# goroda/GPEXP

Hardware: AMD Instinct MI355X
Metric: GP-fit+IVAR-eval points/s at N=32768 d=8 (wall-time in ms_per_step); value = (N+M)/t_step, SURVEY 8d's N/t_fit and M/t_IVAR are points_per_s_fit / points_per_s_ivar right behind it (higher is better)
Workload: dtype f64; 1 GPU; C4: N=32768 d=8 Matern-5/2 (rho=0.5,s=1,noise=0.1) kfill+potrf+potrs+logdet+IVAR over M=32768 MC points; N=32768, d=8, M=32768, kernel=matern52, seed=32768, parallelism=1 GPU

## Files before the change

### gpexp_amd/_lib.py

```python
import ctypes as C
import os

import numpy as np

_HERE = os.path.dirname(os.path.abspath(__file__))
LIB_PATH = os.path.join(_HERE, "libgpx_hip.so")

c_i64 = C.c_int64
c_dp = C.POINTER(C.c_double)
c_ip = C.POINTER(c_i64)
c_vp = C.c_void_p

_SIGS = {
    "gpx_abi_version": (C.c_int, []),
    "gpx_last_error": (C.c_char_p, []),
    "gpx_create": (C.c_int, [C.c_int, C.POINTER(c_vp)]),
    "gpx_destroy": (C.c_int, [c_vp]),
    "gpx_sync": (C.c_int, [c_vp]),
    "gpx_trim": (C.c_int, [c_vp]),
    "gpx_device_info": (C.c_int, [c_vp, C.c_char_p, C.c_int, C.POINTER(C.c_int), c_ip, C.POINTER(C.c_int)]),
    "gpx_mat_from_host": (C.c_int, [c_vp, c_dp, c_i64, c_i64, C.c_int, C.POINTER(c_vp)]),
    "gpx_mat_alloc": (C.c_int, [c_vp, c_i64, c_i64, C.c_int, C.POINTER(c_vp)]),
    "gpx_mat_free": (C.c_int, [c_vp, c_vp]),
    "gpx_mat_clone": (C.c_int, [c_vp, c_vp, C.POINTER(c_vp)]),
# ... 113 lines not shown
    "gpx_dist2_diag_pack": (C.c_int, [c_vp, c_vp, c_i64, c_i64, c_i64, c_vp, c_i64, c_i64]),
    "gpx_dist2_update": (C.c_int, [c_vp, c_vp, c_i64, c_i64, c_i64, c_i64, c_vp, c_i64, c_i64, c_i64, c_i64]),
    "gpx_dist2_update_multi": (C.c_int, [c_vp, c_vp, c_i64, c_i64, c_i64, c_i64, c_i64, C.c_int, C.c_int, C.c_int, C.c_int, c_i64,
                                         C.c_int, C.POINTER(c_vp), c_ip, C.c_int]),
    "gpx_dist2_pack_rows": (C.c_int, [c_vp, c_vp, c_i64, c_i64, c_i64, c_vp, c_i64, c_i64, c_i64, c_i64]),
    "gpx_dist2_pack_diag": (C.c_int, [c_vp, c_vp, c_i64, c_i64, c_i64, c_vp, c_i64]),
    "gpx_program_run": (C.c_int, [c_vp, c_ip, c_i64, c_ip, c_i64, c_dp]),
    "gpx_program_capture": (C.c_int, [c_vp, c_ip, c_i64, c_ip, c_i64, C.POINTER(c_vp)]),
    "gpx_graph_launch": (C.c_int, [c_vp, c_vp, c_dp, c_ip]),
    "gpx_graph_free": (C.c_int, [c_vp, c_vp]),
    "gpx_dist2_unpack_rows": (C.c_int, [c_vp, c_vp, c_i64, c_i64, c_i64, c_i64, c_vp, c_i64, c_i64, c_i64]),
    "gpx_dist2_unpack_diag": (C.c_int, [c_vp, c_vp, c_i64, c_i64, c_i64, c_vp, c_i64]),
    "gpx_dist2_unpack_diag_at": (C.c_int, [c_vp, c_vp, c_i64, c_i64, c_i64, c_vp, c_i64, c_i64]),
    "gpx_dist2_trsv_diag": (C.c_int, [c_vp, c_vp, c_i64, c_i64, c_i64, c_vp, c_i64, C.c_int]),
    "gpx_dist2_gemv": (C.c_int, [c_vp, c_vp, c_i64, c_i64, c_i64, c_i64, c_vp, c_i64, c_vp, c_i64, C.c_int]),
    "gpx_dist2_logdet_acc": (C.c_int, [c_vp, c_vp, c_i64, c_i64, c_i64, c_i64, c_vp]),
    "gpx_stream_select": (C.c_int, [c_vp, C.c_int]),
    "gpx_event_record": (C.c_int, [c_vp, C.c_int]),
    "gpx_event_wait": (C.c_int, [c_vp, C.c_int]),
    "gpx_dist_finish": (C.c_int, [c_vp, c_vp]),
    "gpx_ivar_grad": (C.c_int, [c_vp, C.c_int, C.c_int, c_dp, C.c_int, c_vp, c_vp, c_vp, c_dp, c_dp]),
    "gpx_ivar_grad_w": (C.c_int, [c_vp, C.c_int, C.c_int, c_dp, C.c_int, c_vp, c_vp, c_vp, c_dp, c_vp, c_dp]),
    "gpx_ivar_grad_rows": (C.c_int, [c_vp, C.c_int, C.c_int, c_dp, C.c_int, c_vp, c_vp, c_vp, c_vp, c_i64, c_dp]),
    "gpx_var_grad": (C.c_int, [c_vp, C.c_int, C.c_int, c_dp, C.c_int, c_vp, c_vp, c_vp, c_dp, c_dp, c_dp, c_dp]),
    "gpx_var_grad_newpt": (C.c_int, [c_vp, C.c_int, C.c_int, c_dp, C.c_int, c_vp, c_vp, c_vp, c_dp]),
    "gpx_fitc_var_grad": (C.c_int, [c_vp, c_vp, C.c_int, C.c_int, c_dp, C.c_int, c_vp, c_vp, c_dp, c_dp, c_dp, c_dp]),
    "gpx_fitc_var_grad_newpt": (C.c_int, [c_vp, c_vp, C.c_int, C.c_int, c_dp, C.c_int, c_vp, c_vp, c_dp]),
    "gpx_profile_enable": (C.c_int, [c_vp, C.c_int]),
    "gpx_profile_reset": (C.c_int, [c_vp]),
    "gpx_profile_get": (C.c_int, [c_vp, C.c_int, c_ip, c_dp, c_dp, c_dp]),
    "gpx_dbg_gemm": (C.c_int, [c_vp, c_vp, c_vp, c_vp, C.c_int, C.c_int, C.c_int]),
    "gpx_dbg_gemm_strassen": (C.c_int, [c_vp, c_vp, c_vp, c_vp]),
    "gpx_dbg_gemm_strassen_depth": (C.c_int, [c_vp, c_vp, c_vp, c_vp, C.c_int]),
    "gpx_dbg_gemm_tri": (C.c_int, [c_vp, c_vp, c_vp, c_vp, C.c_int, C.c_int, C.c_int]),
    "gpx_dbg_gemm_ksplit": (C.c_int, [c_vp, c_vp, c_vp, c_vp, C.c_int, C.c_int]),
    "gpx_dbg_kfill_plan": (C.c_int, [c_vp, C.c_int, C.c_int, c_dp, C.c_int, c_vp, c_vp, C.POINTER(C.c_int), c_dp]),
    "gpx_dbg_colreduce_plan": (C.c_int, [c_i64, c_i64, C.POINTER(c_i64), C.POINTER(c_i64)]),
    "gpx_dbg_panel_bcast_plan": (C.c_int, [C.c_int, C.c_int, c_i64, C.c_int, C.POINTER(c_i64), C.POINTER(C.c_int),
                                           C.POINTER(c_i64), c_i64, C.POINTER(c_i64)]),
    "gpx_dbg_guard_violations": (c_i64, [c_vp]),
    "gpx_dbg_guard_selftest": (C.c_int, [c_vp]),
    "gpx_dbg_pool_stats": (C.c_int, [c_vp, C.POINTER(c_i64), C.POINTER(c_i64)]),
    "gpx_dbg_spin": (C.c_int, [c_vp, C.c_int]),
    "gpx_dbg_spin_us": (C.c_int, [c_vp, c_i64]),
    "gpx_dbg_stamp": (C.c_int, [c_vp, C.c_int]),
    "gpx_dbg_spin_until": (C.c_int, [c_vp, C.c_int, c_i64]),
    "gpx_dbg_event_elapsed": (C.c_int, [c_vp, C.c_int, C.c_int, c_dp]),
    "gpx_dbg_leaf_stamps": (C.c_int, [c_vp, c_vp, C.c_int, C.POINTER(c_i64)]),
    "gpx_dbg_greedy_var_scores": (C.c_int, [c_vp, C.c_int, C.c_int, c_dp, C.c_int, c_vp, c_ip, c_i64, c_dp]),
}

_lib = None


def load():
    global _lib
    if _lib is not None:
        return _lib
    path = os.environ.get("GPX_LIB_PATH", LIB_PATH)
    if not os.path.exists(path):
        raise ImportError(
            "gpexp_amd: %s not found - the HIP library is required (no CPU fallback). "
            "Build it with `make -C gpexp_amd/csrc` or __graft_entry__.build()." % path)
    lib = C.CDLL(path)
    for name, (res, args) in _SIGS.items():
        fn = getattr(lib, name)
# ... 43 lines not shown
```

### gpexp_amd/csrc/api.hip

```cpp
#include "gpx_internal.h"
#include <stdarg.h>
#include <stdio.h>
#include <string.h>
#include <math.h>
#include <stdlib.h>

static thread_local char g_err[1024] = "";

void gpx_set_error(const char* fmt, ...) {
  va_list ap;
  va_start(ap, fmt);
  vsnprintf(g_err, sizeof(g_err), fmt, ap);
  va_end(ap);
}

static constexpr int64_t GUARD = 4096;

int gpx_dev_alloc(gpx_ctx* ctx, int64_t bytes, void** out) {
  if (bytes <= 0) bytes = 8;
  bytes = gpx_round_up(bytes, 256);
  const int64_t key = bytes + (ctx->guard ? 2 * GUARD : 0);
  void* base = nullptr;
  auto it = ctx->pool.find(key);
  if (it != ctx->pool.end()) {
// ... 1327 lines not shown
                   : launch_gemm_ksplit_small(ctx, A->p, A->ld, B->p, B->ld, C->p, C->ld, m, n, k, mode == 3, parts, P);
}

int gpx_dbg_gemm(gpx_ctx* ctx, const gpx_mat* A, const gpx_mat* B, gpx_mat* C, int bt, int accumulate, int lower) {
  GPX_ARG(ctx && A && B && C, "NULL argument");
  const int64_t m = C->prows, n = C->pcols, k = A->pcols;
  GPX_ARG(A->prows == m, "A rows");
  GPX_ARG(bt ? (B->prows == n && B->pcols == k) : (B->prows == k && B->pcols == n), "B shape");
  GPX_TRY(launch_gemm(ctx, A->p, A->ld, B->p, B->ld, C->p, C->ld, m, n, k, bt != 0, accumulate != 0,
                      lower != 0));
  GPX_HIP(hipStreamSynchronize(ctx->stream));
  return 0;
}

int gpx_dbg_gemm_strassen(gpx_ctx* ctx, const gpx_mat* A, const gpx_mat* B, gpx_mat* C) {
  GPX_ARG(ctx && A && B && C, "NULL argument");
  const int64_t m = C->prows, n = C->pcols, k = A->pcols;
  GPX_ARG(A->prows == m && B->prows == k && B->pcols == n, "operand shapes");
  GPX_TRY(launch_gemm_strassen(ctx, A->p, A->ld, B->p, B->ld, C->p, C->ld, m, n, k, 1, nullptr, 0));
  GPX_HIP(hipStreamSynchronize(ctx->stream));
  return 0;
}

int gpx_dbg_gemm_strassen_depth(gpx_ctx* ctx, const gpx_mat* A, const gpx_mat* B, gpx_mat* C, int depth) {
  GPX_ARG(ctx && A && B && C, "NULL argument");
  GPX_ARG(depth >= 0 && depth <= GPX_STRASSEN_MAX_DEPTH, "strassen: depth out of range");
  const int64_t m = C->prows, n = C->pcols, k = A->pcols;
  GPX_ARG(A->prows == m && B->prows == k && B->pcols == n, "operand shapes");
  GPX_TRY(launch_gemm_strassen(ctx, A->p, A->ld, B->p, B->ld, C->p, C->ld, m, n, k, depth, nullptr, 0));
  GPX_HIP(hipStreamSynchronize(ctx->stream));
  return 0;
}

}
```

### gpexp_amd/csrc/chol.hip

```cpp
#include "gpx_internal.h"
#include <algorithm>
#include <math.h>
#include <stdlib.h>
#include <stddef.h>

namespace {

constexpr int NB = GPX_TILE;
constexpr int LS = NB + 1;

typedef double d4 __attribute__((ext_vector_type(4)));

__device__ __forceinline__ double readlane_d(double v, int srclane) {
  int lo = __builtin_amdgcn_readlane(__double2loint(v), srclane);
  int hi = __builtin_amdgcn_readlane(__double2hiint(v), srclane);
  return __hiloint2double(hi, lo);
}

constexpr int LB = 16;
constexpr int TS17 = LB + 1;
constexpr int BSZ = LB * TS17;
constexpr int LEAF_CB = LB * LB + 64 + LB;

__device__ __forceinline__ constexpr int sb_off(int I, int J) { return (I * (I + 1) / 2 + J) * BSZ; }
// ... 1249 lines not shown
  const int64_t mid = (b0 + b1) / 2;
  GPX_TRY(trsm_left_oop_rec(ctx, P, b0, mid, B, ldb, W, ldw, m));
  const int64_t r0 = blk_off(P, mid), r1 = blk_off(P, b1), c0 = blk_off(P, b0);
  const int depth = P.strassen ? std::min(P.strassen, strassen_gate(r1 - r0, m, r0 - c0)) : 0;
  if (depth > 0)
    GPX_TRY(launch_gemm_strassen(ctx, P.L + r0 * P.ld + c0, P.ld, W + c0 * ldw, ldw, B + r0 * ldb, ldb, r1 - r0, m, r0 - c0,
                                 depth, P.sscr, P.sscr_bytes));
  else
    GPX_TRY(launch_gemm(ctx, P.L + r0 * P.ld + c0, P.ld, W + c0 * ldw, ldw, B + r0 * ldb, ldb, r1 - r0, m, r0 - c0, false,
                        true, false));
  return trsm_left_oop_rec(ctx, P, mid, b1, B, ldb, W, ldw, m);
}

int chol_trsm_left_oop(gpx_ctx* ctx, gpx_mat* Lm, double* B, int64_t ldb, double* W, int64_t ldw, int64_t m) {
  GPX_ARG(Lm && Lm->factored && Lm->aux && B && W && B != W, "trsm: matrix has not been factored / bad buffers");
  if (m == 0) return 0;
  GPX_TRY(chol_binv_ensure(ctx, Lm));
  PotrsPlan P;
  P.L = Lm->p;
  P.ld = Lm->ld;
  P.n = Lm->prows;
  P.sib = Lm->binv_ib;
  P.ib = P.sib < 1024 ? P.sib : 1024;
  P.nblk = (P.n + P.ib - 1) / P.ib;
  P.binv = Lm->binv;
  P.binvT = nullptr;
  P.part = nullptr;
  void* ps = nullptr;
  int64_t sbytes = 0;
  int depth = 0;
  const int64_t max_depth = env_i64("GPX_STRASSEN", GPX_STRASSEN_MAX_DEPTH);
  if (P.nblk >= 2 && max_depth > 0) {
    const int64_t r0 = blk_off(P, P.nblk / 2);
    for (depth = (int)std::min<int64_t>(max_depth, strassen_gate(P.n - r0, m, r0)); depth > 0; --depth) {
      sbytes = gemm_strassen_scratch_bytes(P.n - r0, m, r0, depth);
      if (sbytes > 0 && gpx_dev_alloc(ctx, sbytes, &ps) == 0) break;
      (void)hipGetLastError();
      ps = nullptr;
    }
  }
  P.strassen = ps ? depth : 0;
  P.sscr = (double*)ps;
  P.sscr_bytes = sbytes;
  const int r = trsm_left_oop_rec(ctx, P, 0, P.nblk, B, ldb, W, ldw, m);
  if (ps) {
    (void)hipStreamSynchronize(ctx->stream);
    gpx_dev_release(ctx, ps, sbytes);
  }
  return r;
}

int chol_trsm_left_group(gpx_ctx* ctx, const double* Lg, int64_t ld, const double* invd, int64_t w, int64_t below, int64_t ib,
                         double* B, int64_t ldb, int64_t m, double* inv, double* tmp, double* W, int64_t ldw) {
  GPX_ARG(Lg && invd && B && inv && tmp && W && W != B && w > 0 && w % NB == 0 && ib >= NB && ib % NB == 0, "trsm group: bad arguments");
  if (m == 0) return 0;
  GPX_TRY(binv_build_range(ctx, Lg, ld, invd, inv, ib, w, tmp));
  PotrsPlan P;
  P.L = Lg;
  P.ld = ld;
  P.n = w;
  P.ib = P.sib = ib;
  P.nblk = (w + ib - 1) / ib;
  P.binv = inv;
  P.binvT = nullptr;
  P.part = nullptr;
  GPX_TRY(trsm_left_oop_rec(ctx, P, 0, P.nblk, B, ldb, W, ldw, m));
  if (below > 0) GPX_TRY(launch_gemm(ctx, Lg + w * ld, ld, W, ldw, B + w * ldb, ldb, below, m, w, false, true, false));
  return gpx_copy2d(ctx, W, ldw, B, ldb, w, m);
}
// ... 66 lines not shown
```

### gpexp_amd/csrc/gemm_f64.hip

```cpp
#include "gpx_internal.h"
#include <stdlib.h>

namespace {

typedef double d4 __attribute__((ext_vector_type(4)));

constexpr int KB = 16;
constexpr int SA = KB + 1;

template <bool BT, int TE>
struct Smem {
  double a[2][TE * SA];
  double b[2][BT ? TE * SA : KB * (TE + 16)];
};

template <bool LOWER>
__device__ __forceinline__ bool tile_of(int sblk, int within, int tiles_m, int tiles_n, int sb_cols, int sb_shift,
                                        int* by, int* bx, int rot = 0) {
  const int sbm = (1 << sb_shift) - 1;
  int sr, sc;
  if (LOWER) {
    const int nsr = (tiles_m + sbm) >> sb_shift;
    const int noff = nsr * (nsr - 1) / 2;
    if (sblk < noff) {
// ... 397 lines not shown
  gemm_tile<false, true, TE, NoSeg, Multi>(sm, A, lda, B, ldb, dst.c[0], ldc, nk, by, bx, NoSeg(), dst);
}

template <bool BSIDE>
__global__ __launch_bounds__(256) void strassen_sums_kernel(const double* __restrict__ X, int64_t ldx, int64_t hr, int64_t hc,
                                                            double* __restrict__ S, int64_t lds, int64_t sstride) {
  const int64_t j = ((int64_t)blockIdx.x * 256 + threadIdx.x) * 2;
  if (j >= hc) return;
  for (int64_t i = blockIdx.y; i < hr; i += gridDim.y) {
    const double* x1 = X + i * ldx + j;
    const double* x2 = X + (i + hr) * ldx + j;
    const double2 x11 = *reinterpret_cast<const double2*>(x1);
    const double2 x12 = *reinterpret_cast<const double2*>(x1 + hc);
    const double2 x21 = *reinterpret_cast<const double2*>(x2);
    const double2 x22 = *reinterpret_cast<const double2*>(x2 + hc);
    double* o = S + i * lds + j;
#define GPX_S2(k_, ex_, ey_) *reinterpret_cast<double2*>(o + (k_) * sstride) = make_double2(ex_, ey_)
    GPX_S2(0, x11.x + x22.x, x11.y + x22.y);
    if (BSIDE) {
      GPX_S2(1, x12.x - x22.x, x12.y - x22.y);
      GPX_S2(2, x21.x - x11.x, x21.y - x11.y);
      GPX_S2(3, x11.x + x12.x, x11.y + x12.y);
      GPX_S2(4, x21.x + x22.x, x21.y + x22.y);
    } else {
      GPX_S2(1, x21.x + x22.x, x21.y + x22.y);
      GPX_S2(2, x11.x + x12.x, x11.y + x12.y);
      GPX_S2(3, x21.x - x11.x, x21.y - x11.y);
      GPX_S2(4, x12.x - x22.x, x12.y - x22.y);
    }
#undef GPX_S2
  }
}

template <bool BT, bool ACC>
__global__ __launch_bounds__(256, 2) void gemm_f64_batched_kernel(const double* A, int64_t lda, int64_t sa,
                                                                  const double* B, int64_t ldb, int64_t sb, double* C,
                                                                  int64_t ldc, int64_t sc, int nk, int tiles_n, int hiprio) {
  __shared__ Smem<BT, 64> sm;
  if (hiprio) __builtin_amdgcn_s_setprio(3);
  const int64_t b = blockIdx.y;
  const int by = blockIdx.x / tiles_n, bx = blockIdx.x - by * tiles_n;
  gemm_tile<BT, ACC, 64>(sm, A + b * sa, lda, B + b * sb, ldb, C + b * sc, ldc, nk, by, bx);
}

template <bool LOWER>
__global__ __launch_bounds__(256, 2) void gemm_f64_ksplit_kernel(const double* A, int64_t lda, const double* B, int64_t ldb,
                                                                 double* P, int64_t n, int64_t sp, int nk_slice, int parts,
                                                                 int tiles_m, int tiles_n, int sb_cols, int sb_shift) {
  __shared__ Smem<true, 128> sm;
  const int w = blockIdx.x, xcd = w & 7, q = w >> 3, sbs2 = 2 * sb_shift;
  const int job = (q >> sbs2) * 8 + xcd, within = q & ((1 << sbs2) - 1);
  int sb, slice;
  if (LOWER) {
    const int nsr = (tiles_m + (1 << sb_shift) - 1) >> sb_shift, noff = nsr * (nsr - 1) / 2;
    if (job < parts * noff) {
      slice = job / noff;
      sb = job - slice * noff;
    } else {
      const int jj = job - parts * noff;
      slice = jj / nsr;
      sb = noff + jj - slice * nsr;
    }
  } else {
    const int nsb = ((tiles_m + (1 << sb_shift) - 1) >> sb_shift) * sb_cols;
    slice = job / nsb;
    sb = job - slice * nsb;
// ... 273 lines not shown
  return 0;
}

static int launch_gemm_multi(gpx_ctx* ctx, const double* A, int64_t lda, const double* B, int64_t ldb, const Multi& dst,
                             int64_t ldc, int64_t m, int64_t n, int64_t k) {
  GPX_ARG(m % 128 == 0 && n % 128 == 0 && k % KB == 0 && k > 0 && m > 0 && n > 0, "gemm: m,n must be multiples of 128 and k of 16");
  GPX_ARG((lda % 2) == 0 && (ldb % 2) == 0, "gemm: leading dimensions must be even (16-byte loads)");
  GPX_ARG(dst.nd >= 1 && dst.nd <= GPX_MULTI_MAX, "gemm: bad destination count");
  const double tiles128 = (double)(m / 128) * (double)(n / 128);
  const int te = tiles128 < 1024.0 ? 64 : 128;
  const Plan p = make_plan(m, n, false, te);
  GPX_ARG(p.wgs < ((int64_t)1 << 31), "gemm: grid too large");
  const int nk = (int)(k / KB);
  ProfScope ps(ctx, GPX_PROF_GEMM, 2.0 * (double)m * (double)n * (double)k, 0.0);
  if (te == 64)
    hipLaunchKernelGGL(gemm_f64_multi_kernel<64>, dim3((unsigned)p.wgs), dim3(256), 0, ctx->stream, A, lda, B, ldb, dst, ldc, nk,
                       p.tm, p.tn, p.sbc, p.sb_shift);
  else
    hipLaunchKernelGGL(gemm_f64_multi_kernel<128>, dim3((unsigned)p.wgs), dim3(256), 0, ctx->stream, A, lda, B, ldb, dst, ldc, nk,
                       p.tm, p.tn, p.sbc, p.sb_shift);
  GPX_HIP(hipGetLastError());
  return 0;
}

static inline bool strassen_shape_ok(int64_t m, int64_t n, int64_t k, int depth) {
  return depth >= 1 && depth <= GPX_STRASSEN_MAX_DEPTH && m > 0 && n > 0 && k > 0 && m % ((int64_t)128 << depth) == 0 &&
         n % ((int64_t)128 << depth) == 0 && k % ((int64_t)KB << depth) == 0;
}

static inline int64_t strassen_level_elems(int64_t hm, int64_t hn, int64_t hk) {
  return 5 * (hm * gpx_skew_ld(hk) + hk * gpx_skew_ld(hn));
}

int64_t gemm_strassen_scratch_bytes(int64_t m, int64_t n, int64_t k, int depth) {
  if (!strassen_shape_ok(m, n, k, depth)) return 0;
  int64_t elems = 0;
  for (int d = 0; d < depth; ++d) {
    m /= 2, n /= 2, k /= 2;
    elems += strassen_level_elems(m, n, k);
  }
  return elems * 8;
}

namespace {
struct SDest {
  double* c;
  double s;
};
struct SProd {
  int a, b, nq, q[2];
  double s[2];
};
constexpr SProd kStrassen[7] = {
    {-1, -1, 2, {0, 3}, {1.0, 1.0}},
    {-2, 0, 2, {2, 3}, {1.0, -1.0}},
    {0, -2, 2, {1, 3}, {1.0, 1.0}},
    {3, -3, 2, {0, 2}, {1.0, 1.0}},
    {-3, 3, 2, {1, 0}, {1.0, -1.0}},
    {-4, -4, 1, {3, 0}, {1.0, 0.0}},
    {-5, -5, 1, {0, 0}, {1.0, 0.0}},
};
}

static int strassen_rec(gpx_ctx* ctx, const double* A, int64_t lda, const double* B, int64_t ldb, const SDest* dst, int nd,
                        int64_t ldc, int64_t m, int64_t n, int64_t k, int depth, double* scratch) {
  if (depth == 0) {
    for (int d = 1; d < nd; ++d)
      for (int e = 0; e < d; ++e) GPX_ARG(dst[d].c != dst[e].c, "strassen: two destinations of one product coincide");
    if (nd == 1 && dst[0].s == 1.0) return launch_gemm(ctx, A, lda, B, ldb, dst[0].c, ldc, m, n, k, false, true, false);
    if (nd == 2 && dst[0].s == 1.0) return launch_gemm_dual(ctx, A, lda, B, ldb, dst[0].c, dst[1].c, dst[1].s, ldc, m, n, k);
    GPX_ARG(nd >= 1 && nd <= GPX_MULTI_MAX, "strassen: too many destinations for one product");
    Multi md;
    for (int d = 0; d < GPX_MULTI_MAX; ++d) {
      md.c[d] = d < nd ? dst[d].c : nullptr;
      md.s[d] = d < nd ? dst[d].s : 0.0;
    }
    md.nd = nd;
    return launch_gemm_multi(ctx, A, lda, B, ldb, md, ldc, m, n, k);
  }
  const int64_t hm = m / 2, hn = n / 2, hk = k / 2, lsa = gpx_skew_ld(hk), lsb = gpx_skew_ld(hn);
  const int64_t sa = hm * lsa, sb = hk * lsb;
  double* const S = scratch;
  double* const T = scratch + 5 * sa;
  double* const below = T + 5 * sb;
  {
    ProfScope ps(ctx, GPX_PROF_REDUCE, 5.0 * (double)hm * hk + 5.0 * (double)hk * hn, 72.0 * ((double)hm * hk + (double)hk * hn));
    hipLaunchKernelGGL(strassen_sums_kernel<false>, dim3((unsigned)((hk / 2 + 255) / 256), (unsigned)(hm < 65535 ? hm : 65535)),
                       dim3(256), 0, ctx->stream, A, lda, hm, hk, S, lsa, sa);
    hipLaunchKernelGGL(strassen_sums_kernel<true>, dim3((unsigned)((hn / 2 + 255) / 256), (unsigned)(hk < 65535 ? hk : 65535)),
                       dim3(256), 0, ctx->stream, B, ldb, hk, hn, T, lsb, sb);
    if (hipGetLastError() != hipSuccess) {
      gpx_set_error("strassen: operand-sum launch failed");
      return -2;
    }
  }
  const int64_t qoff[4] = {0, hn, hm * ldc, hm * ldc + hn};
  for (const SProd& p : kStrassen) {
    const double* Ap = p.a < 0 ? S + (-1 - p.a) * sa : (p.a == 0 ? A : A + hm * lda + hk);
    const double* Bp = p.b < 0 ? T + (-1 - p.b) * sb : (p.b == 0 ? B : B + hk * ldb + hn);
    SDest sub[GPX_MULTI_MAX];
    int ns = 0;
    for (int d = 0; d < nd; ++d)
      for (int j = 0; j < p.nq; ++j) {
        GPX_ARG(ns < GPX_MULTI_MAX, "strassen: too many destinations for one product");
        sub[ns++] = SDest{dst[d].c + qoff[p.q[j]], dst[d].s * p.s[j]};
      }
    GPX_TRY(strassen_rec(ctx, Ap, p.a < 0 ? lsa : lda, Bp, p.b < 0 ? lsb : ldb, sub, ns, ldc, hm, hn, hk, depth - 1, below));
  }
  return 0;
}

int launch_gemm_strassen(gpx_ctx* ctx, const double* A, int64_t lda, const double* B, int64_t ldb, double* C, int64_t ldc,
                         int64_t m, int64_t n, int64_t k, int depth, double* scratch, int64_t scratch_bytes) {
  if (depth > GPX_STRASSEN_MAX_DEPTH) depth = GPX_STRASSEN_MAX_DEPTH;
  if ((lda % 2) != 0 || (ldb % 2) != 0 || C == A || C == B) depth = 0;
  void* own = nullptr;
  int64_t need = 0;
  for (; depth > 0; --depth) {
    need = gemm_strassen_scratch_bytes(m, n, k, depth);
    if (need == 0) continue;
    if (scratch && scratch_bytes >= need) break;
    if (gpx_dev_alloc(ctx, need, &own) == 0) {
      scratch = (double*)own;
      break;
    }
    (void)hipGetLastError();
    own = nullptr;
  }
  if (depth <= 0) return launch_gemm(ctx, A, lda, B, ldb, C, ldc, m, n, k, false, true, false);
  const SDest top{C, 1.0};
  const int r = strassen_rec(ctx, A, lda, B, ldb, &top, 1, ldc, m, n, k, depth, scratch);
  if (own) {
    (void)hipStreamSynchronize(ctx->stream);
    gpx_dev_release(ctx, own, need);
  }
  return r;
}

int launch_dist2_update(gpx_ctx* ctx, double* C, int64_t ldc, int64_t lr0, int64_t m, int64_t lc0, int64_t n, int64_t nb, int Pr,
                        int Pc, int pr, int pc, int64_t piece_stride, int64_t dsz, int nseg, const double* const* g,
                        const int64_t* ks, int below_diag) {
  if (m == 0 || n == 0 || nseg == 0) return 0;
  GPX_ARG(nseg > 0 && nseg <= GPX_SEG_MAX && Pr >= 1 && Pr <= GPX_MAX_PR && Pc >= 1, "dist2 update: too many segments / grid rows");
  GPX_ARG(m % 128 == 0 && n % 128 == 0 && nb % 128 == 0 && lr0 % nb == 0 && lc0 % nb == 0 && (ldc % 2) == 0, "dist2 update: alignment");
  Dist2Upd u;
  for (int s = 0; s < nseg; ++s) {
    u.g[s] = g[s];
    for (int p = 0; p < Pr; ++p) u.li0[s][p] = (int)(ks[s] + 1 <= p ? 0 : (ks[s] - p) / Pr + 1);
  }
  u.nseg = nseg;
  u.seg_nk = (int)(nb / KB);
  u.Pr = Pr; u.Pc = Pc; u.pr = pr; u.pc = pc;
  u.nb = (int)nb;
  u.gld = (int)gpx_g_ld(nb);
  u.li_first = (int)(lr0 / nb);
  u.lj_first = (int)(lc0 / nb);
  u.below_diag = below_diag;
  u.piece_stride = piece_stride;
  u.dsz = dsz;
  double tiles128 = 0.0;
  for (int64_t lj = lc0 / nb; lj * nb < lc0 + n; ++lj) {
    const int64_t J = lj * Pc + pc;
    const int64_t cw = (lc0 + n - lj * nb) < nb ? (lc0 + n - lj * nb) : nb;
    for (int64_t li = lr0 / nb; li * nb < lr0 + m; ++li) {
// ... 56 lines not shown
```

### gpexp_amd/csrc/gpx_internal.h

```cpp
#pragma once
#include <hip/hip_runtime.h>
#include <stdint.h>
#include <stdlib.h>
#include <string>
#include <vector>
#include <map>
#include <memory>
#include <unordered_set>
#include "../../include/gpx.h"
#include "../../include/gpx_dist.h"
#include "../../include/gpx_debug.h"

#define GPX_TILE 128
#define GPX_MAXD GPX_MAX_DIM
#define GPX_NSTREAMS 6
#define GPX_SEG_MAX 8
#ifndef GPX_G_SKEW
#define GPX_G_SKEW 0
#endif
#define GPX_MAX_PR 4

void gpx_set_error(const char* fmt, ...);
#define GPX_HIP(call)                                                                   \
  do {                                                                                  \
// ... 215 lines not shown
    else if ((kind_) == GPX_K_MATERN32) GPX_SE_DISPATCH(GPX_K_MATERN32, d_, CALL); \
    else GPX_SE_DISPATCH(GPX_K_MATERN52, d_, CALL);                             \
  } while (0)

extern "C" __attribute__((visibility("hidden"))) int64_t gpx_eval_chunk(int64_t np);
int gpx_posterior_chunk(gpx_ctx* ctx, const KParams& kp, const gpx_mat* L, const gpx_mat* X, const double* Zc, int64_t mc,
                        double* B, double* Wout, const double* alpha_dev, double* mean_dev, double* mean_host, double* ssq,
                        double* kd, double* part);

int launch_kfill(gpx_ctx* ctx, const KParams& kp, const double* A, int64_t na, const double* B, int64_t nb,
                 int symmetric, const double* d_nugget, int64_t nugget_len, double nugget_scalar,
                 double* out, int64_t prows, int64_t pcols, int64_t ld);
int launch_kfill_offset(gpx_ctx* ctx, const KParams& kp, const double* X, int64_t n, int64_t row_off, int64_t col_off,
                        const double* d_nugget, int64_t nugget_len, double nugget_scalar, double* out, int64_t prows,
                        int64_t pcols, int64_t ld);
int launch_kdiag(gpx_ctx* ctx, const KParams& kp, const double* Z, int64_t m, double* out);
int launch_kfill_cyclic(gpx_ctx* ctx, const KParams& kp, const double* X, int64_t n, const double* d_nugget,
                        int64_t nugget_len, double nugget_scalar, double* out, int64_t prows, int64_t pcols, int64_t ld,
                        int64_t nb, int Pr, int pr, int Pc, int pc);
int gpx_copy2d(gpx_ctx* ctx, const double* src, int64_t lds_, double* dst, int64_t ldd, int64_t rows, int64_t cols);
int gpx_copy2d_lower(gpx_ctx* ctx, const double* src, int64_t lds_, double* dst, int64_t ldd, int64_t n);
int launch_kfill_rows(gpx_ctx* ctx, const KParams& kp, const double* X, int64_t n, int64_t row0, const double* d_nugget,
                      int64_t nugget_len, double nugget_scalar, double* out, int64_t prows_band, int64_t pcols,
                      int64_t ld);

static inline int gpx_chain_prio(const gpx_ctx* ctx) { return ctx->stream == ctx->streams[1] ? 1 : 0; }
int launch_gemm(gpx_ctx* ctx, const double* A, int64_t lda, const double* B, int64_t ldb, double* C, int64_t ldc,
                int64_t m, int64_t n, int64_t k, bool bt, bool accumulate, bool lower);

int launch_gemm_tri(gpx_ctx* ctx, const double* A, int64_t lda, const double* B, int64_t ldb, double* C, int64_t ldc,
                    int64_t m, int64_t n, int64_t k, bool bt, bool accumulate, bool lower, int tri);
constexpr int GPX_STRASSEN_MAX_DEPTH = 2;
int64_t gemm_strassen_scratch_bytes(int64_t m, int64_t n, int64_t k, int depth);
int launch_gemm_strassen(gpx_ctx* ctx, const double* A, int64_t lda, const double* B, int64_t ldb, double* C, int64_t ldc,
                         int64_t m, int64_t n, int64_t k, int depth, double* scratch, int64_t scratch_bytes);
int launch_gemm_ksplit(gpx_ctx* ctx, const double* A, int64_t lda, const double* B, int64_t ldb, double* C, int64_t ldc,
                       int64_t m, int64_t n, int64_t k, bool lower, int64_t parts, double* P, bool assign = false);
int launch_gemm_ksplit_small(gpx_ctx* ctx, const double* A, int64_t lda, const double* B, int64_t ldb, double* C, int64_t ldc,
                             int64_t m, int64_t n, int64_t k, bool assign, int64_t parts, double* P);
int launch_gemm_batched(gpx_ctx* ctx, const double* A, int64_t lda, int64_t sa, const double* B, int64_t ldb, int64_t sb,
                        double* C, int64_t ldc, int64_t sc, int64_t m, int64_t n, int64_t k, bool bt, bool accumulate,
                        int64_t batch);

int launch_dist2_update(gpx_ctx* ctx, double* C, int64_t ldc, int64_t lr0, int64_t m, int64_t lc0, int64_t n, int64_t nb, int Pr,
                        int Pc, int pr, int pc, int64_t piece_stride, int64_t dsz, int nseg, const double* const* g,
                        const int64_t* ks, int below_diag);

int launch_leaf(gpx_ctx* ctx, double* A, int64_t ld, double* inv, int64_t base_index, int64_t n_valid);
int chol_potrf(gpx_ctx* ctx, double* A, int64_t ld, int64_t n, double* invd, int64_t n_valid);
int chol_potrf_nozero(gpx_ctx* ctx, double* A, int64_t ld, int64_t n, double* invd, int64_t base, int64_t n_valid);
int chol_trsm_right(gpx_ctx* ctx, const double* L, int64_t ldl, const double* invd, double* X, int64_t ldx,
                    int64_t m, int64_t n);
int chol_trsm_right_n(gpx_ctx* ctx, const double* L, int64_t ldl, const double* invd, double* X, int64_t ldx,
                      int64_t m, int64_t n);
int chol_trsm_left(gpx_ctx* ctx, const double* L, int64_t ldl, const double* invd, double* B, int64_t ldb,
                   int64_t n, int64_t m);
int chol_trsv(gpx_ctx* ctx, const double* L, int64_t ld, const double* invd, double* y, int64_t n, bool transposed);
int64_t chol_trsv_scratch_bytes(int64_t n);
int chol_trsv_with_scratch(gpx_ctx* ctx, const double* L, int64_t ld, const double* invd, double* y, int64_t n,
                           bool transposed, double* scratch);
int launch_logdet(gpx_ctx* ctx, const double* L, int64_t ld, int64_t n, double* d_out);
int chol_trtri(gpx_ctx* ctx, const gpx_mat* L, double* Linv, double* tmp);
int chol_binv_ensure(gpx_ctx* ctx, gpx_mat* L);
int chol_trsm_right_trailing(gpx_ctx* ctx, gpx_mat* L, int64_t r0, double* X, int64_t ldx, int64_t m, int transposed, double* T);
int chol_trsm_right_leading(gpx_ctx* ctx, gpx_mat* L, int64_t ncols, double* X, int64_t ldx, int64_t m, double* T, int64_t tcap);
int chol_trsm_right_n_leading(gpx_ctx* ctx, gpx_mat* L, int64_t ncols, double* X, int64_t ldx, int64_t m, double* T);
// ... 49 lines not shown
```

### gpexp_amd/device.py

```python
import ctypes as C
import atexit
import os

import numpy as np

from . import _lib
from ._lib import check, as_f64, dptr, c_vp, c_i64, GpxError

K_SE, K_MATERN32, K_MATERN52, K_MEHLER = 0, 1, 2, 3
PROF_CLASSES = ["kfill", "gemm", "leaf", "trsv", "reduce", "greedy", "comm", "kcross"]

_ctx = None


class Context:

    def __init__(self, device=None):
        self.lib = _lib.load()
        if device is None:
            device = int(os.environ.get("LOCAL_RANK", "0"))
        h = c_vp()
        rc = self.lib.gpx_create(int(device), C.byref(h))
        if rc != 0:
            raise RuntimeError("gpexp_amd needs an MI355X: " + self.lib.gpx_last_error().decode())
# ... 769 lines not shown


def var_grad_newpt(ctx, spec, L, X, Z):
    out = np.empty(Z.shape[0] * spec.d)
    check(ctx.lib.gpx_var_grad_newpt(ctx.h, *spec.args(), L.h, X.h, Z.h, dptr(out)))
    return out


def kfill_plan(ctx, spec, X, Z=None):
    ex = C.c_int()
    cen = np.zeros(spec.d)
    check(ctx.lib.gpx_dbg_kfill_plan(ctx.h, *spec.args(), X.h, Z.h if Z is not None else None, C.byref(ex), dptr(cen)))
    return bool(ex.value), cen


def dbg_gemm_tri(ctx, A, B, Cm, bt, accumulate, tri):
    check(ctx.lib.gpx_dbg_gemm_tri(ctx.h, A.h, B.h, Cm.h, int(bt), int(accumulate), int(tri)))


def dbg_gemm_ksplit(ctx, A, B, Cm, mode, parts):
    check(ctx.lib.gpx_dbg_gemm_ksplit(ctx.h, A.h, B.h, Cm.h, int(mode), int(parts)))


def dbg_gemm(ctx, A, B, Cm, bt, accumulate, lower=False):
    check(ctx.lib.gpx_dbg_gemm(ctx.h, A.h, B.h, Cm.h, int(bt), int(accumulate), int(lower)))


def dbg_gemm_strassen(ctx, A, B, Cm):
    check(ctx.lib.gpx_dbg_gemm_strassen(ctx.h, A.h, B.h, Cm.h))


def dbg_gemm_strassen_depth(ctx, A, B, Cm, depth):
    check(ctx.lib.gpx_dbg_gemm_strassen_depth(ctx.h, A.h, B.h, Cm.h, int(depth)))
```

### include/gpx_debug.h

```cpp
#ifndef GPX_DEBUG_H
#define GPX_DEBUG_H
#include "gpx.h"
#ifdef __cplusplus
extern "C" {
#endif

int gpx_dbg_gemm(gpx_ctx* ctx, const gpx_mat* A, const gpx_mat* B, gpx_mat* C, int bt, int accumulate, int lower);
int gpx_dbg_gemm_tri(gpx_ctx* ctx, const gpx_mat* A, const gpx_mat* B, gpx_mat* C, int bt, int accumulate, int tri);
int gpx_dbg_gemm_ksplit(gpx_ctx* ctx, const gpx_mat* A, const gpx_mat* B, gpx_mat* C, int mode, int parts);
int gpx_dbg_gemm_strassen(gpx_ctx* ctx, const gpx_mat* A, const gpx_mat* B, gpx_mat* C);
int gpx_dbg_gemm_strassen_depth(gpx_ctx* ctx, const gpx_mat* A, const gpx_mat* B, gpx_mat* C, int depth);
int gpx_dbg_spin(gpx_ctx* ctx, int ms);
int64_t gpx_dbg_guard_violations(gpx_ctx* ctx);
int gpx_dbg_pool_stats(gpx_ctx* ctx, int64_t* pooled_bytes, int64_t* outstanding_bytes);
int gpx_dbg_guard_selftest(gpx_ctx* ctx);
int gpx_dbg_panel_bcast_plan(int W, int me, int64_t small_elems, int npieces, const int64_t* counts, const int* roots,
                             int64_t* ops, int64_t max_ops, int64_t* nops);
int gpx_dbg_colreduce_plan(int64_t rows, int64_t pcols, int64_t* nchunk, int64_t* bound_elems);
int gpx_dbg_kfill_plan(gpx_ctx* ctx, int kind, int d, const double* hyp, int nhyp, const gpx_mat* X, const gpx_mat* Z,
                       int* exact, double* center);

int gpx_dbg_spin_us(gpx_ctx* ctx, int64_t us);
int gpx_dbg_stamp(gpx_ctx* ctx, int slot);
int gpx_dbg_spin_until(gpx_ctx* ctx, int slot, int64_t us);
int gpx_dbg_event_elapsed(gpx_ctx* ctx, int id0, int id1, double* ms);

int gpx_dbg_leaf_stamps(gpx_ctx* ctx, gpx_mat* K, int fast, int64_t* out30);

int gpx_dbg_greedy_var_scores(gpx_ctx* ctx, int kind, int d, const double* hyp, int nhyp, const gpx_mat* C, const int64_t* keep,
                              int64_t nkeep, double* out_d );

#ifdef __cplusplus
}
#endif
#endif
```

Measured before the change: 105,300 points/s.

## Add one-pass depth-2 Strassen that precomputes all operand sums in one kernel

Adds a one-pass form of two-level Strassen. A single kernel per operand computes all 45 quarter-block sums of A and B up front, then the 49 leaf products run directly from those sums, replacing the recursive two-pass scheme with its intermediate level. A ladder picks the first form whose scratch fits, and it is used in the potrs trsm and the strassen gemm path. The one-pass form needs more scratch memory (45 quarter blocks per operand), so it falls back to two-pass or plain gemm when allocation fails.

```diff
diff --git a/gpexp_amd/_lib.py b/gpexp_amd/_lib.py
--- a/gpexp_amd/_lib.py
+++ b/gpexp_amd/_lib.py
@@ -169,6 +169,11 @@
     "gpx_dbg_gemm": (C.c_int, [c_vp, c_vp, c_vp, c_vp, C.c_int, C.c_int, C.c_int]),
     "gpx_dbg_gemm_strassen": (C.c_int, [c_vp, c_vp, c_vp, c_vp]),
     "gpx_dbg_gemm_strassen_depth": (C.c_int, [c_vp, c_vp, c_vp, c_vp, C.c_int]),
+    "gpx_dbg_gemm_strassen_view": (C.c_int, [c_vp, c_vp, c_i64, c_i64, c_vp, c_i64, c_i64, c_vp, c_i64, c_i64, c_i64, c_i64, c_i64,
+                                             C.c_int]),
+    "gpx_dbg_strassen_forms": (C.c_int, [c_i64, c_i64, c_i64, C.c_int, C.c_int, c_i64, C.POINTER(c_i64), C.POINTER(C.c_int),
+                                         C.POINTER(C.c_int)]),
+    "gpx_dbg_strassen_scratch_bytes": (c_i64, [c_i64, c_i64, c_i64, C.c_int]),
     "gpx_dbg_gemm_tri": (C.c_int, [c_vp, c_vp, c_vp, c_vp, C.c_int, C.c_int, C.c_int]),
     "gpx_dbg_gemm_ksplit": (C.c_int, [c_vp, c_vp, c_vp, c_vp, C.c_int, C.c_int]),
     "gpx_dbg_kfill_plan": (C.c_int, [c_vp, C.c_int, C.c_int, c_dp, C.c_int, c_vp, c_vp, C.POINTER(C.c_int), c_dp]),
diff --git a/gpexp_amd/csrc/api.hip b/gpexp_amd/csrc/api.hip
--- a/gpexp_amd/csrc/api.hip
+++ b/gpexp_amd/csrc/api.hip
@@ -1383,4 +1383,36 @@
   return 0;
 }
 
-}
+int gpx_dbg_gemm_strassen_view(gpx_ctx* ctx, const gpx_mat* A, int64_t ar0, int64_t ac0, const gpx_mat* B, int64_t br0, int64_t bc0,
+                               gpx_mat* C, int64_t cr0, int64_t cc0, int64_t m, int64_t n, int64_t k, int depth) {
+  GPX_ARG(ctx && A && B && C, "NULL argument");
+  GPX_ARG(depth >= 0 && depth <= GPX_STRASSEN_MAX_DEPTH, "strassen: depth out of range");
+  GPX_ARG(m > 0 && n > 0 && k > 0 && ar0 >= 0 && ac0 >= 0 && br0 >= 0 && bc0 >= 0 && cr0 >= 0 && cc0 >= 0, "view: negative extent / offset");
+  GPX_ARG(ar0 + m <= A->prows && ac0 + k <= A->pcols && br0 + k <= B->prows && bc0 + n <= B->pcols && cr0 + m <= C->prows &&
+              cc0 + n <= C->pcols, "view: outside its matrix");
+  GPX_ARG(ac0 % 2 == 0 && bc0 % 2 == 0 && cc0 % 2 == 0 && A->ld % 2 == 0 && B->ld % 2 == 0 && C->ld % 2 == 0,
+          "view: column offsets and leading dimensions must be even (16-byte accesses)");
+  GPX_TRY(launch_gemm_strassen(ctx, A->p + ar0 * A->ld + ac0, A->ld, B->p + br0 * B->ld + bc0, B->ld, C->p + cr0 * C->ld + cc0, C->ld,
+                               m, n, k, depth, nullptr, 0));
+  GPX_HIP(hipStreamSynchronize(ctx->stream));
+  return 0;
+}
+
+int gpx_dbg_strassen_forms(int64_t m, int64_t n, int64_t k, int max_depth, int allow_onepass, int64_t avail_bytes, int64_t* forms9,
+                           int* nforms, int* first_fit) {
+  GPX_ARG(forms9 && nforms && first_fit, "NULL argument");
+  StrassenForm f[GPX_STRASSEN_MAX_DEPTH + 1];
+  const int nf = gemm_strassen_ladder(m, n, k, max_depth, allow_onepass != 0, f);
+  for (int i = 0; i < nf; ++i) {
+    forms9[3 * i] = f[i].depth;
+    forms9[3 * i + 1] = f[i].onepass;
+    forms9[3 * i + 2] = f[i].bytes;
+  }
+  *nforms = nf;
+  *first_fit = gemm_strassen_first_fit(f, nf, avail_bytes);
+  return 0;
+}
+
+int64_t gpx_dbg_strassen_scratch_bytes(int64_t m, int64_t n, int64_t k, int depth) { return gemm_strassen_scratch_bytes(m, n, k, depth); }
+
+}
diff --git a/gpexp_amd/csrc/chol.hip b/gpexp_amd/csrc/chol.hip
--- a/gpexp_amd/csrc/chol.hip
+++ b/gpexp_amd/csrc/chol.hip
@@ -1305,9 +1305,13 @@
   const int64_t max_depth = env_i64("GPX_STRASSEN", GPX_STRASSEN_MAX_DEPTH);
   if (P.nblk >= 2 && max_depth > 0) {
     const int64_t r0 = blk_off(P, P.nblk / 2);
-    for (depth = (int)std::min<int64_t>(max_depth, strassen_gate(P.n - r0, m, r0)); depth > 0; --depth) {
-      sbytes = gemm_strassen_scratch_bytes(P.n - r0, m, r0, depth);
-      if (sbytes > 0 && gpx_dev_alloc(ctx, sbytes, &ps) == 0) break;
+    StrassenForm forms[GPX_STRASSEN_MAX_DEPTH + 1];
+    const int nf = gemm_strassen_ladder(P.n - r0, m, r0, (int)std::min<int64_t>(max_depth, strassen_gate(P.n - r0, m, r0)),
+                                        gemm_strassen_onepass_enabled(), forms);
+    for (int f = 0; f < nf; ++f) {
+      sbytes = forms[f].bytes;
+      depth = forms[f].depth;
+      if (gpx_dev_alloc(ctx, sbytes, &ps) == 0) break;
       (void)hipGetLastError();
       ps = nullptr;
     }
diff --git a/gpexp_amd/csrc/gemm_f64.hip b/gpexp_amd/csrc/gemm_f64.hip
--- a/gpexp_amd/csrc/gemm_f64.hip
+++ b/gpexp_amd/csrc/gemm_f64.hip
@@ -453,6 +453,61 @@
   }
 }
 
+template <bool BSIDE>
+__device__ __forceinline__ void strassen_sums5(const double2& x11, const double2& x12, const double2& x21, const double2& x22,
+                                               double2 (&o)[5]) {
+  o[0] = make_double2(x11.x + x22.x, x11.y + x22.y);
+  if (BSIDE) {
+    o[1] = make_double2(x12.x - x22.x, x12.y - x22.y);
+    o[2] = make_double2(x21.x - x11.x, x21.y - x11.y);
+    o[3] = make_double2(x11.x + x12.x, x11.y + x12.y);
+    o[4] = make_double2(x21.x + x22.x, x21.y + x22.y);
+  } else {
+    o[1] = make_double2(x21.x + x22.x, x21.y + x22.y);
+    o[2] = make_double2(x11.x + x12.x, x11.y + x12.y);
+    o[3] = make_double2(x21.x - x11.x, x21.y - x11.y);
+    o[4] = make_double2(x12.x - x22.x, x12.y - x22.y);
+  }
+}
+
+constexpr int GPX_SUMS2_BLOCKS = 45;
+template <bool BSIDE>
+__global__ __launch_bounds__(256) void strassen_sums2_kernel(const double* __restrict__ X, int64_t ldx, int64_t qr, int64_t qc,
+                                                             double* __restrict__ O, int64_t ldo, int64_t bs) {
+  const int64_t j = ((int64_t)blockIdx.x * 256 + threadIdx.x) * 2;
+  if (j >= qc) return;
+  for (int64_t i = blockIdx.y; i < qr; i += gridDim.y) {
+    double2 x[4][4];
+#pragma unroll
+    for (int r = 0; r < 4; ++r)
+#pragma unroll
+      for (int c = 0; c < 4; ++c) x[r][c] = *reinterpret_cast<const double2*>(X + (r * qr + i) * ldx + c * qc + j);
+    double* o = O + i * ldo + j;
+#define GPX_S2(k_, v_) *reinterpret_cast<double2*>(o + (k_) * bs) = (v_)
+    double2 y[2][2][5];
+#pragma unroll
+    for (int u = 0; u < 2; ++u)
+#pragma unroll
+      for (int v = 0; v < 2; ++v) strassen_sums5<BSIDE>(x[u][v], x[u][2 + v], x[2 + u][v], x[2 + u][2 + v], y[u][v]);
+    double2 t[5];
+#pragma unroll
+    for (int s = 0; s < 5; ++s) {
+      strassen_sums5<BSIDE>(y[0][0][s], y[0][1][s], y[1][0][s], y[1][1][s], t);
+#pragma unroll
+      for (int e = 0; e < 5; ++e) GPX_S2(7 * s + e, t[e]);
+      GPX_S2(7 * s + 5, y[0][0][s]);
+      GPX_S2(7 * s + 6, y[1][1][s]);
+    }
+#pragma unroll
+    for (int h = 0; h < 2; ++h) {
+      strassen_sums5<BSIDE>(x[2 * h][2 * h], x[2 * h][2 * h + 1], x[2 * h + 1][2 * h], x[2 * h + 1][2 * h + 1], t);
+#pragma unroll
+      for (int e = 0; e < 5; ++e) GPX_S2(35 + 5 * h + e, t[e]);
+    }
+#undef GPX_S2
+  }
+}
+
 template <bool BT, bool ACC>
 __global__ __launch_bounds__(256, 2) void gemm_f64_batched_kernel(const double* A, int64_t lda, int64_t sa,
                                                                   const double* B, int64_t ldb, int64_t sb, double* C,
@@ -792,7 +847,7 @@
   return 5 * (hm * gpx_skew_ld(hk) + hk * gpx_skew_ld(hn));
 }
 
-int64_t gemm_strassen_scratch_bytes(int64_t m, int64_t n, int64_t k, int depth) {
+int64_t gemm_strassen_scratch_bytes_twopass(int64_t m, int64_t n, int64_t k, int depth) {
   if (!strassen_shape_ok(m, n, k, depth)) return 0;
   int64_t elems = 0;
   for (int d = 0; d < depth; ++d) {
@@ -800,6 +855,34 @@
     elems += strassen_level_elems(m, n, k);
   }
   return elems * 8;
+}
+
+int64_t gemm_strassen_scratch_bytes(int64_t m, int64_t n, int64_t k, int depth) {
+  if (depth != 2) return gemm_strassen_scratch_bytes_twopass(m, n, k, depth);
+  if (!strassen_shape_ok(m, n, k, depth)) return 0;
+  const int64_t qm = m / 4, qn = n / 4, qk = k / 4;
+  return 8 * GPX_SUMS2_BLOCKS * (qm * gpx_skew_ld(qk) + qk * gpx_skew_ld(qn));
+}
+
+bool gemm_strassen_onepass_enabled() {
+  const char* e = getenv("GPX_STRASSEN_ONEPASS");
+  return !(e && *e) || atoll(e) != 0;
+}
+
+int gemm_strassen_ladder(int64_t m, int64_t n, int64_t k, int max_depth, bool allow_onepass, StrassenForm out[GPX_STRASSEN_MAX_DEPTH + 1]) {
+  int cnt = 0;
+  for (int depth = std::min(max_depth, GPX_STRASSEN_MAX_DEPTH); depth > 0; --depth) {
+    if (!strassen_shape_ok(m, n, k, depth)) continue;
+    if (depth == 2 && allow_onepass) out[cnt++] = StrassenForm{2, 1, gemm_strassen_scratch_bytes(m, n, k, 2)};
+    out[cnt++] = StrassenForm{depth, 0, gemm_strassen_scratch_bytes_twopass(m, n, k, depth)};
+  }
+  return cnt;
+}
+
+int gemm_strassen_first_fit(const StrassenForm* forms, int nf, int64_t bytes) {
+  int f = 0;
+  while (f < nf && forms[f].bytes > bytes) ++f;
+  return f;
 }
 
 namespace {
@@ -822,6 +905,16 @@
 };
 }
 
+static int strassen_expand(const SDest* dst, int nd, const SProd& p, const int64_t* qoff, SDest* sub, int* ns) {
+  *ns = 0;
+  for (int d = 0; d < nd; ++d)
+    for (int j = 0; j < p.nq; ++j) {
+      GPX_ARG(*ns < GPX_MULTI_MAX, "strassen: too many destinations for one product");
+      sub[(*ns)++] = SDest{dst[d].c + qoff[p.q[j]], dst[d].s * p.s[j]};
+    }
+  return 0;
+}
+
 static int strassen_rec(gpx_ctx* ctx, const double* A, int64_t lda, const double* B, int64_t ldb, const SDest* dst, int nd,
                         int64_t ldc, int64_t m, int64_t n, int64_t k, int depth, double* scratch) {
   if (depth == 0) {
@@ -860,12 +953,53 @@
     const double* Bp = p.b < 0 ? T + (-1 - p.b) * sb : (p.b == 0 ? B : B + hk * ldb + hn);
     SDest sub[GPX_MULTI_MAX];
     int ns = 0;
-    for (int d = 0; d < nd; ++d)
-      for (int j = 0; j < p.nq; ++j) {
-        GPX_ARG(ns < GPX_MULTI_MAX, "strassen: too many destinations for one product");
-        sub[ns++] = SDest{dst[d].c + qoff[p.q[j]], dst[d].s * p.s[j]};
-      }
+    GPX_TRY(strassen_expand(dst, nd, p, qoff, sub, &ns));
     GPX_TRY(strassen_rec(ctx, Ap, p.a < 0 ? lsa : lda, Bp, p.b < 0 ? lsb : ldb, sub, ns, ldc, hm, hn, hk, depth - 1, below));
+  }
+  return 0;
+}
+
+static int strassen_onepass2(gpx_ctx* ctx, const double* A, int64_t lda, const double* B, int64_t ldb, const SDest* dst, int nd,
+                             int64_t ldc, int64_t m, int64_t n, int64_t k, double* scratch) {
+  const int64_t qm = m / 4, qn = n / 4, qk = k / 4, loa = gpx_skew_ld(qk), lob = gpx_skew_ld(qn);
+  const int64_t ba = qm * loa, bb = qk * lob;
+  double* const SA = scratch;
+  double* const SB = scratch + GPX_SUMS2_BLOCKS * ba;
+  {
+    ProfScope ps(ctx, GPX_PROF_REDUCE, 45.0 * ((double)qm * qk + (double)qk * qn), 8.0 * 61.0 * ((double)qm * qk + (double)qk * qn));
+    hipLaunchKernelGGL(strassen_sums2_kernel<false>, dim3((unsigned)((qk / 2 + 255) / 256), (unsigned)(qm < 65535 ? qm : 65535)),
+                       dim3(256), 0, ctx->stream, A, lda, qm, qk, SA, loa, ba);
+    hipLaunchKernelGGL(strassen_sums2_kernel<true>, dim3((unsigned)((qn / 2 + 255) / 256), (unsigned)(qk < 65535 ? qk : 65535)),
+                       dim3(256), 0, ctx->stream, B, ldb, qk, qn, SB, lob, bb);
+    if (hipGetLastError() != hipSuccess) {
+      gpx_set_error("strassen: operand-sum launch failed");
+      return -2;
+    }
+  }
+  auto operand = [](int x1, int x2, const double* X, int64_t ldx, int64_t qr, int64_t qc, const double* S, int64_t ldo, int64_t bs,
+                    int64_t* ld) -> const double* {
+    if (x1 >= 0 && x2 >= 0) {
+      *ld = ldx;
+      return X + (x1 == 0 ? 0 : 2 * (qr * ldx + qc)) + (x2 == 0 ? 0 : qr * ldx + qc);
+    }
+    *ld = ldo;
+    if (x1 < 0) return S + (7 * (-1 - x1) + (x2 < 0 ? -1 - x2 : (x2 == 0 ? 5 : 6))) * bs;
+    return S + (35 + 5 * (x1 == 0 ? 0 : 1) + (-1 - x2)) * bs;
+  };
+  const int64_t qoff1[4] = {0, 2 * qn, 2 * qm * ldc, 2 * qm * ldc + 2 * qn}, qoff2[4] = {0, qn, qm * ldc, qm * ldc + qn};
+  for (const SProd& p : kStrassen) {
+    SDest sub1[GPX_MULTI_MAX];
+    int n1 = 0;
+    GPX_TRY(strassen_expand(dst, nd, p, qoff1, sub1, &n1));
+    for (const SProd& q : kStrassen) {
+      SDest sub2[GPX_MULTI_MAX];
+      int n2 = 0;
+      GPX_TRY(strassen_expand(sub1, n1, q, qoff2, sub2, &n2));
+      int64_t la, lb;
+      const double* Ap = operand(p.a, q.a, A, lda, qm, qk, SA, loa, ba, &la);
+      const double* Bp = operand(p.b, q.b, B, ldb, qk, qn, SB, lob, bb, &lb);
+      GPX_TRY(strassen_rec(ctx, Ap, la, Bp, lb, sub2, n2, ldc, qm, qn, qk, 0, nullptr));
+    }
   }
   return 0;
 }
@@ -876,20 +1010,26 @@
   if ((lda % 2) != 0 || (ldb % 2) != 0 || C == A || C == B) depth = 0;
   void* own = nullptr;
   int64_t need = 0;
-  for (; depth > 0; --depth) {
-    need = gemm_strassen_scratch_bytes(m, n, k, depth);
-    if (need == 0) continue;
-    if (scratch && scratch_bytes >= need) break;
-    if (gpx_dev_alloc(ctx, need, &own) == 0) {
-      scratch = (double*)own;
-      break;
-    }
-    (void)hipGetLastError();
-    own = nullptr;
-  }
-  if (depth <= 0) return launch_gemm(ctx, A, lda, B, ldb, C, ldc, m, n, k, false, true, false);
+  StrassenForm forms[GPX_STRASSEN_MAX_DEPTH + 1];
+  const int nf = gemm_strassen_ladder(m, n, k, depth, gemm_strassen_onepass_enabled(), forms);
+  int f = 0;
+  if (scratch) {
+    f = gemm_strassen_first_fit(forms, nf, scratch_bytes);
+  } else {
+    for (; f < nf; ++f) {
+      need = forms[f].bytes;
+      if (gpx_dev_alloc(ctx, need, &own) == 0) {
+        scratch = (double*)own;
+        break;
+      }
+      (void)hipGetLastError();
+      own = nullptr;
+    }
+  }
+  if (f >= nf) return launch_gemm(ctx, A, lda, B, ldb, C, ldc, m, n, k, false, true, false);
   const SDest top{C, 1.0};
-  const int r = strassen_rec(ctx, A, lda, B, ldb, &top, 1, ldc, m, n, k, depth, scratch);
+  const int r = forms[f].onepass ? strassen_onepass2(ctx, A, lda, B, ldb, &top, 1, ldc, m, n, k, scratch)
+                                 : strassen_rec(ctx, A, lda, B, ldb, &top, 1, ldc, m, n, k, forms[f].depth, scratch);
   if (own) {
     (void)hipStreamSynchronize(ctx->stream);
     gpx_dev_release(ctx, own, need);
diff --git a/gpexp_amd/csrc/gpx_internal.h b/gpexp_amd/csrc/gpx_internal.h
--- a/gpexp_amd/csrc/gpx_internal.h
+++ b/gpexp_amd/csrc/gpx_internal.h
@@ -271,6 +271,15 @@
                     int64_t m, int64_t n, int64_t k, bool bt, bool accumulate, bool lower, int tri);
 constexpr int GPX_STRASSEN_MAX_DEPTH = 2;
 int64_t gemm_strassen_scratch_bytes(int64_t m, int64_t n, int64_t k, int depth);
+int64_t gemm_strassen_scratch_bytes_twopass(int64_t m, int64_t n, int64_t k, int depth);
+bool gemm_strassen_onepass_enabled();
+struct StrassenForm {
+  int depth;
+  int onepass;
+  int64_t bytes;
+};
+int gemm_strassen_ladder(int64_t m, int64_t n, int64_t k, int max_depth, bool allow_onepass, StrassenForm out[GPX_STRASSEN_MAX_DEPTH + 1]);
+int gemm_strassen_first_fit(const StrassenForm* forms, int nf, int64_t bytes);
 int launch_gemm_strassen(gpx_ctx* ctx, const double* A, int64_t lda, const double* B, int64_t ldb, double* C, int64_t ldc,
                          int64_t m, int64_t n, int64_t k, int depth, double* scratch, int64_t scratch_bytes);
 int launch_gemm_ksplit(gpx_ctx* ctx, const double* A, int64_t lda, const double* B, int64_t ldb, double* C, int64_t ldc,
diff --git a/gpexp_amd/device.py b/gpexp_amd/device.py
--- a/gpexp_amd/device.py
+++ b/gpexp_amd/device.py
@@ -825,3 +825,8 @@
 
 def dbg_gemm_strassen_depth(ctx, A, B, Cm, depth):
     check(ctx.lib.gpx_dbg_gemm_strassen_depth(ctx.h, A.h, B.h, Cm.h, int(depth)))
+
+
+def dbg_gemm_strassen_view(ctx, A, a0, B, b0, Cm, c0, m, n, k, depth):
+    check(ctx.lib.gpx_dbg_gemm_strassen_view(ctx.h, A.h, int(a0[0]), int(a0[1]), B.h, int(b0[0]), int(b0[1]), Cm.h, int(c0[0]),
+                                             int(c0[1]), int(m), int(n), int(k), int(depth)))
diff --git a/include/gpx_debug.h b/include/gpx_debug.h
--- a/include/gpx_debug.h
+++ b/include/gpx_debug.h
@@ -10,6 +10,11 @@
 int gpx_dbg_gemm_ksplit(gpx_ctx* ctx, const gpx_mat* A, const gpx_mat* B, gpx_mat* C, int mode, int parts);
 int gpx_dbg_gemm_strassen(gpx_ctx* ctx, const gpx_mat* A, const gpx_mat* B, gpx_mat* C);
 int gpx_dbg_gemm_strassen_depth(gpx_ctx* ctx, const gpx_mat* A, const gpx_mat* B, gpx_mat* C, int depth);
+int gpx_dbg_gemm_strassen_view(gpx_ctx* ctx, const gpx_mat* A, int64_t ar0, int64_t ac0, const gpx_mat* B, int64_t br0, int64_t bc0,
+                               gpx_mat* C, int64_t cr0, int64_t cc0, int64_t m, int64_t n, int64_t k, int depth);
+int gpx_dbg_strassen_forms(int64_t m, int64_t n, int64_t k, int max_depth, int allow_onepass, int64_t avail_bytes, int64_t* forms9,
+                           int* nforms, int* first_fit);
+int64_t gpx_dbg_strassen_scratch_bytes(int64_t m, int64_t n, int64_t k, int depth);
 int gpx_dbg_spin(gpx_ctx* ctx, int ms);
 int64_t gpx_dbg_guard_violations(gpx_ctx* ctx);
 int gpx_dbg_pool_stats(gpx_ctx* ctx, int64_t* pooled_bytes, int64_t* outstanding_bytes);
```

Result: no change. 105,600 points/s (median of 6 runs) (+0.3%).
